# Eclectic-Sheep/sheeprl

Hardware: NVIDIA H100
Metric: Dreamer-V3 train-steps/sec (S, bs16 seq64 horizon15, 64x64x3 obs) (higher is better)
Workload: dtype f32

## Files before the change

include/b200rl.h:

```cpp
#ifndef B200RL_H_
#define B200RL_H_

#include <cuda_runtime_api.h>

#ifdef __cplusplus
extern "C" {
#endif

const char* b200rl_last_error(void);
int b200rl_abi_version(void);
const char* b200rl_build_arch(void);
int b200rl_device_check(void);

int b200rl_gemm_f32(const float* A, const float* B, float* C, const float* bias, int M, int N, int K, int lda, int ldb,
                    int ldc, int transA, int transB, int accumulate, cudaStream_t stream);
int b200rl_set_matmul_precision(int tf32_passes);
int b200rl_get_matmul_precision(void);
int b200rl_gemm_tc_supported(const float* A, const float* B, int M, int N, int K, int lda, int ldb, int transA,
                             int transB);
int b200rl_gemm_tc(const float* A, const float* B, float* C, const float* bias, int M, int N, int K, int lda, int ldb,
                   int ldc, int transA, int transB, int accumulate, cudaStream_t stream);
int b200rl_tf32_split(const float* X, float* Xhi, float* Xlo, long long n, cudaStream_t stream);
int b200rl_tf32_split_t(const float* W, float* Thi, float* Tlo, int rows, int cols, long long ldw, long long ldt,
                        cudaStream_t stream);
int b200rl_gemm_tc_presplit_supported(const float* A, const float* Bhi, const float* Blo, int M, int N, int K, int lda,
                                      int ldb);
int b200rl_gemm_tc_presplit(const float* A, const float* Bhi, const float* Blo, float* C, const float* bias, int M, int N,
                            int K, int lda, int ldb, int ldc, int accumulate, cudaStream_t stream);
int b200rl_gemm_ln_supported(const float* A, const float* W, int M, int N, int K, int lda, int ldw, int mode);
int b200rl_gemm_ln(const float* A, const float* W, int M, int N, int K, int lda, int ldw, const float* gamma,
                   const float* beta, float eps, int act, float* pre, long long ldpre, float* out, long long ldout,
                   int mode, const float* h_prev, long long ldh, float* h_out, long long ldho, float* h_out2,
                   long long ldho2, cudaStream_t stream);
int b200rl_gemm_ln_presplit_supported(const float* A, const float* Whi, const float* Wlo, int M, int N, int K, int lda,
                                      int ldw, int mode);
int b200rl_gemm_ln_presplit(const float* A, const float* Whi, const float* Wlo, int M, int N, int K, int lda, int ldw,
                            const float* gamma, const float* beta, float eps, int act, float* pre, long long ldpre,
                            float* out, long long ldout, int mode, const float* h_prev, long long ldh, float* h_out,
                            long long ldho, float* h_out2, long long ldho2, cudaStream_t stream);
int b200rl_ln_act_route(int C, long long ld0, long long ld1, long long ld2, const float* p0, const float* p1,
                        const float* p2, const float* gamma, const float* beta);
int b200rl_ln_act_fwd(const float* X, const float* gamma, const float* beta, float* Y, long long M, int C,
                      long long ldx, long long ldy, float eps, int act, cudaStream_t stream);
int b200rl_ln_act_bwd(const float* X, const float* gamma, const float* beta, const float* dY, float* dX, float* dgamma,
                      float* dbeta, long long M, int C, long long ldx, long long lddy, long long lddx, float eps,
                      int act, int accumulate, cudaStream_t stream);
int b200rl_col_sum(const float* X, float* out, long long M, int C, long long ldx, int accumulate, cudaStream_t stream);

int b200rl_obs_prep(const void* obs_nchw, int is_uint8, float* out_nhwc, long long NB, int C, int HW,
                    cudaStream_t stream);
int b200rl_transpose_batched(const float* X, float* Y, int NB, int a, int b, cudaStream_t stream);
int b200rl_transpose2d(const float* X, float* Y, int rows, int cols, long long ldx, long long ldy, cudaStream_t stream);
int b200rl_conv_down(const float* big, const float* W, float* small_, int NB, int h, int w, int Cs, int Cb,
                     cudaStream_t stream);
int b200rl_conv_up(const float* small_, const float* W, float* big, const float* bias, int NB, int h, int w, int Cs,
                   int Cb, cudaStream_t stream);
int b200rl_conv_wgrad(const float* small_, const float* big, float* dW, int NB, int h, int w, int Cs, int Cb,
// ... 224 lines not shown
```

sheeprl_b200/csrc/gemm_tc.cu:

```cuda
#include <cuda.h>
#include <cudaTypedefs.h>

#include <mutex>
#include <unordered_map>

#include "common.cuh"

namespace {

constexpr int BM = 128, BK = 32;
constexpr int NTHREADS = 384;
constexpr int NSPLIT_THREADS = 96;
constexpr int NCONS_WARPS = 8;
constexpr int PRODUCER_REGS = 56, CONSUMER_REGS = 224;
template <int PASSES, bool PRESPLIT> __host__ __device__ constexpr int b_buffers() { return PRESPLIT ? (PASSES == 3 ? 2 : 1) : 3; }
template <int BN, int PASSES, bool PRESPLIT> constexpr int stages_for() {
  return (227 * 1024 - 1024 - 256) / ((BM + b_buffers<PASSES, PRESPLIT>() * BN) * BK * (int)sizeof(float));
}

__device__ __forceinline__ uint32_t smem_u32(const void* p) { return (uint32_t)__cvta_generic_to_shared(p); }

__device__ __forceinline__ void mbar_init(uint64_t* bar, uint32_t count) {
  asm volatile("mbarrier.init.shared::cta.b64 [%0], %1;" ::"r"(smem_u32(bar)), "r"(count) : "memory");
}
__device__ __forceinline__ void mbar_expect_tx(uint64_t* bar, uint32_t bytes) {
  asm volatile("mbarrier.arrive.expect_tx.shared::cta.b64 _, [%0], %1;" ::"r"(smem_u32(bar)), "r"(bytes) : "memory");
}
__device__ __forceinline__ void mbar_arrive(uint64_t* bar) {
  asm volatile("mbarrier.arrive.shared::cta.b64 _, [%0];" ::"r"(smem_u32(bar)) : "memory");
}
__device__ __forceinline__ bool mbar_try_wait(uint64_t* bar, uint32_t parity) {
  uint32_t ok;
  asm volatile(
      "{\n\t"
      ".reg .pred p;\n\t"
      "mbarrier.try_wait.parity.shared::cta.b64 p, [%1], %2;\n\t"
      "selp.u32 %0, 1, 0, p;\n\t"
      "}"
// ... 479 lines not shown
  *bw = w < 128 ? w : 128;
  int rest = 128 / *bw;
  *bh = h < rest ? h : rest;
  *bn = rest / *bh;
  return (w % *bw == 0) && (h % *bh == 0) && (*bw * *bh * *bn == 128) && (NB % *bn == 0);
}

static unsigned persistent_grid_y(int tiles, unsigned gz) {
  const long long total = (long long)tiles * gz;
  if (total <= 2LL * kNumSMs) return (unsigned)tiles;
  unsigned gy = kNumSMs / gz;
  if (gy < 1) gy = 1;
  return gy < (unsigned)tiles ? gy : (unsigned)tiles;
}

__device__ __forceinline__ float tf32_hi(float x) { return __uint_as_float(__float_as_uint(x) & 0xffffe000u); }
__device__ __forceinline__ void store_split(float* P, float* L, long long i, float v) {
  if (L) { const float h = tf32_hi(v); P[i] = h; L[i] = v - h; }
  else P[i] = v;
}

__global__ void tf32_split_kernel(const float* __restrict__ X, float* __restrict__ H, float* __restrict__ L, long long n) {
  const long long i = ((long long)blockIdx.x * blockDim.x + threadIdx.x) * 4;
  if (i + 4 <= n && !((reinterpret_cast<uintptr_t>(X) | reinterpret_cast<uintptr_t>(H) | reinterpret_cast<uintptr_t>(L)) & 15)) {
    const float4 v = *reinterpret_cast<const float4*>(X + i);
    const float4 h = make_float4(tf32_hi(v.x), tf32_hi(v.y), tf32_hi(v.z), tf32_hi(v.w));
    *reinterpret_cast<float4*>(H + i) = h;
    *reinterpret_cast<float4*>(L + i) = make_float4(v.x - h.x, v.y - h.y, v.z - h.z, v.w - h.w);
  } else {
    for (long long j = i; j < i + 4 && j < n; ++j) store_split(H, L, j, X[j]);
  }
}

__global__ void tf32_split_t_kernel(const float* __restrict__ W, float* __restrict__ H, float* __restrict__ L, int rows,
                                    int cols, long long ldw, long long ldt) {
  __shared__ float t[32][33];
  const int c0 = blockIdx.x * 32, r0 = blockIdx.y * 32;
  for (int j = threadIdx.y; j < 32; j += blockDim.y) {
    const int r = r0 + j, c = c0 + threadIdx.x;
    t[j][threadIdx.x] = (r < rows && c < cols) ? W[(long long)r * ldw + c] : 0.f;
  }
  __syncthreads();
  for (int j = threadIdx.y; j < 32; j += blockDim.y) {
    const int c = c0 + j, r = r0 + threadIdx.x;
    if (c < cols && r < ldt) store_split(H, L, (long long)c * ldt + r, t[threadIdx.x][j]);
  }
}

__global__ void conv_pack_down_kernel(const float* __restrict__ W, float* __restrict__ P, float* __restrict__ L, int Cs,
                                      int Cb) {
  const long long idx = (long long)blockIdx.x * blockDim.x + threadIdx.x;
  if (idx >= (long long)Cs * Cb * 16) return;
  const int cb = (int)(idx % Cb);
  const int tap = (int)((idx / Cb) % 16);
  const int cs = (int)(idx / ((long long)Cb * 16));
  store_split(P, L, idx, W[((long long)cs * Cb + cb) * 16 + tap]);
}
__global__ void conv_pack_up_kernel(const float* __restrict__ W, float* __restrict__ P, float* __restrict__ L, int Cs,
                                    int Cb) {
  const long long idx = (long long)blockIdx.x * blockDim.x + threadIdx.x;
  if (idx >= (long long)Cs * Cb * 16) return;
  const int cs = (int)(idx % Cs);
  const int t = (int)((idx / Cs) % 4);
  const int cb = (int)((idx / ((long long)Cs * 4)) % Cb);
  const int par = (int)(idx / ((long long)Cs * 4 * Cb));
  const int py = par >> 1, px = par & 1;
// ... 170 lines not shown
  RL_CHECK_ARG(W && Whi && Wlo, "null pointer");
  return conv_pack_impl(W, Whi, Wlo, mode_up, Cs, Cb, st);
}
extern "C" int b200rl_conv_down_tc(const float* big, const float* Wpacked, float* small_, int NB, int h, int w, int Cs,
                                   int Cb, cudaStream_t st) {
  RL_CHECK_ARG(big && Wpacked && small_, "null pointer");
  RL_CHECK_ARG(b200rl_conv_tc_supported(0, NB, h, w, Cs, Cb), "shape not eligible for the tensor-core conv path");
  return launch_conv(MODE_DOWN, big, Wpacked, nullptr, small_, nullptr, NB, h, w, Cb, Cs, st);
}
extern "C" int b200rl_conv_up_tc(const float* small_, const float* Wpacked, float* big, const float* bias, int NB, int h,
                                 int w, int Cs, int Cb, cudaStream_t st) {
  RL_CHECK_ARG(big && Wpacked && small_, "null pointer");
  RL_CHECK_ARG(b200rl_conv_tc_supported(1, NB, h, w, Cs, Cb), "shape not eligible for the tensor-core conv path");
  return launch_conv(MODE_UP, small_, Wpacked, nullptr, big, bias, NB, h, w, Cs, Cb, st);
}
extern "C" int b200rl_conv_down_tc_presplit(const float* big, const float* Whi, const float* Wlo, float* small_, int NB,
                                            int h, int w, int Cs, int Cb, cudaStream_t st) {
  RL_CHECK_ARG(big && Whi && Wlo && small_, "null pointer");
  RL_CHECK_ARG(b200rl_conv_tc_supported(0, NB, h, w, Cs, Cb), "shape not eligible for the tensor-core conv path");
  return launch_conv(MODE_DOWN, big, Whi, Wlo, small_, nullptr, NB, h, w, Cb, Cs, st);
}
extern "C" int b200rl_conv_up_tc_presplit(const float* small_, const float* Whi, const float* Wlo, float* big,
                                          const float* bias, int NB, int h, int w, int Cs, int Cb, cudaStream_t st) {
  RL_CHECK_ARG(big && Whi && Wlo && small_, "null pointer");
  RL_CHECK_ARG(b200rl_conv_tc_supported(1, NB, h, w, Cs, Cb), "shape not eligible for the tensor-core conv path");
  return launch_conv(MODE_UP, small_, Whi, Wlo, big, bias, NB, h, w, Cs, Cb, st);
}

extern "C" int b200rl_tf32_split(const float* X, float* Xhi, float* Xlo, long long n, cudaStream_t st) {
  RL_CHECK_ARG(X && Xhi && Xlo, "null pointer");
  RL_CHECK_ARG(n >= 0, "negative length");
  if (n == 0) return B200RL_OK;
  tf32_split_kernel<<<ceil_div((n + 3) / 4, 256), 256, 0, st>>>(X, Xhi, Xlo, n);
  RL_CHECK_LAUNCH();
  return B200RL_OK;
}
extern "C" int b200rl_tf32_split_t(const float* W, float* Thi, float* Tlo, int rows, int cols, long long ldw, long long ldt,
                                   cudaStream_t st) {
  RL_CHECK_ARG(W && Thi && Tlo, "null pointer");
  RL_CHECK_ARG(rows > 0 && cols > 0 && ldw >= cols && ldt >= rows, "bad transposed-split geometry");
  dim3 grid(ceil_div(cols, 32), ceil_div(ldt, 32));
  tf32_split_t_kernel<<<grid, dim3(32, 8), 0, st>>>(W, Thi, Tlo, rows, cols, ldw, ldt);
  RL_CHECK_LAUNCH();
  return B200RL_OK;
}

extern "C" int b200rl_gemm_tc_supported(const float* A, const float* B, int M, int N, int K, int lda, int ldb,
                                        int transA, int transB) {
  (void)transA; (void)transB;
  if (M < 32 || N < 48 || K < 32) return 0;
  if ((lda & 3) || (ldb & 3)) return 0;
  if ((reinterpret_cast<uintptr_t>(A) & 15) || (reinterpret_cast<uintptr_t>(B) & 15)) return 0;
  return 1;
}

namespace {
struct FusedTail { float* part; int ks, mpad, ldw; };

int gemm_tc_impl(const float* A, const float* B, const float* Blo, float* C, const float* bias, int M, int N, int K,
                 int lda, int ldb, int ldc, int transA, int transB, int accumulate, cudaStream_t st, FusedTail* fused) {
  RL_CHECK_ARG(A && B && (C || fused), "null pointer");
  RL_CHECK_ARG(b200rl_gemm_tc_supported(A, B, M, N, K, lda, ldb, transA, transB), "shape not eligible for the tensor-core path");
  RL_CHECK_ARG(!Blo || (transB && !(reinterpret_cast<uintptr_t>(Blo) & 15)), "pre-split B must be 16-byte aligned [N][K] planes");
  const int BN = (N <= 64) ? 64 : 128;
  CUtensorMap ma, mb, mb2;
  if (!transA) { if (int rc = get_map(A, M, K, lda, BM, &ma)) return rc; }
// ... 249 lines not shown
```

sheeprl_b200/engine.py:

```python
from __future__ import annotations

import math
from typing import Dict, Mapping, Optional, Sequence

import torch

from sheeprl_b200.params import FlatGroup

ACT_NONE, ACT_SILU = 0, 1
TWOHOT_LOW, TWOHOT_HIGH = -20.0, 20.0


def decoder_channels(cfg, in_channels: int, cnn_dims: Optional[Mapping[str, int]] = None) -> int:
    a = cfg.algo
    dec = list(a.cnn_keys.decoder or [])
    if dec == list(a.cnn_keys.encoder or []):
        return in_channels
    missing = [k for k in dec if k not in (cnn_dims or {})]
    if missing:
        raise ValueError(f"the channel count of the decoded image key(s) {missing} is not known (pass cnn_dims)")
    return sum(int(cnn_dims[k]) for k in dec)


def check_decoder_keys(cfg) -> None:
# ... 89 lines not shown
    return wm, actor, critic, dict(chans=chans, dch=dch, E=E, Ev=Ev, stages=stages)


def _check_supported_modules(cfg) -> None:
    a, w = cfg.algo, cfg.algo.world_model
    blocks = {"algo": a, "encoder": w.encoder, "observation_model": w.observation_model, "reward_model": w.reward_model,
              "discount_model": w.discount_model, "transition_model": w.transition_model,
              "representation_model": w.representation_model, "recurrent_model": w.recurrent_model, "actor": a.actor,
              "critic": a.critic}
    for name, blk in blocks.items():
        for key in ("dense_act", "cnn_act"):
            v = blk.get(key, None)
            if v is not None and not str(v).endswith("SiLU"):
                raise NotImplementedError(f"{name}.{key} = {v}: only torch.nn.SiLU is built")
        for key in ("layer_norm", "mlp_layer_norm", "cnn_layer_norm"):
            v = blk.get(key, None)
            if v is not None and "LayerNorm" not in str(v.get("cls", "LayerNorm")):
                raise NotImplementedError(f"{name}.{key}.cls = {v.get('cls')}: only the LayerNorm variants are built")
    for name in ("reward_model", "discount_model"):
        blk = blocks[name]
        if int(blk.get("dense_units", a.dense_units)) != int(a.dense_units) or int(blk.get("mlp_layers", a.mlp_layers)) != int(a.mlp_layers):
            raise NotImplementedError(f"world_model.{name}: dense_units / mlp_layers must equal algo.dense_units / algo.mlp_layers")
    if int(w.observation_model.get("cnn_channels_multiplier", w.encoder.cnn_channels_multiplier)) != int(w.encoder.cnn_channels_multiplier):
        raise NotImplementedError("observation_model.cnn_channels_multiplier must equal encoder.cnn_channels_multiplier")
    for name in ("actor", "critic"):
        blk = blocks[name]
        if int(blk.get("dense_units", a.dense_units)) != int(a.dense_units) or int(blk.get("mlp_layers", a.mlp_layers)) != int(a.mlp_layers):
            raise NotImplementedError(f"algo.{name}: dense_units / mlp_layers must equal algo.dense_units / algo.mlp_layers")


FUSED_DENSE_MAX_ROWS = 4096


def dense_ln_act(ops, x, W, gamma, beta, eps, act, out, pre=None, scratch=None):
    if x.shape[0] <= FUSED_DENSE_MAX_ROWS and ops.gemm_ln_supported(x, W):
        ops.gemm_ln_act(x, W, gamma, beta, eps, act, out, pre)
        return
    tmp = pre if pre is not None else scratch
    ops.gemm(x, W, tmp, False, True)
    ops.ln_act_fwd(tmp, gamma, beta, eps, act, out)


class _MLP:

    def __init__(self, eng, group: FlatGroup, prefix: str, in_dim: int, hidden: int, n_hidden: int,
                 out_dim: Optional[int], rows: int, eps: float, tag: str, train: bool):
        self.eng, self.g, self.prefix = eng, group, prefix
        self.in_dim, self.hidden, self.n_hidden, self.out_dim, self.eps = in_dim, hidden, n_hidden, out_dim, eps
        self.rows = rows
        new = eng._buf
        self.pre = [new(f"{tag}.pre{i}", rows, hidden) for i in range(n_hidden)]
        self.act = [new(f"{tag}.act{i}", rows, hidden) for i in range(n_hidden)]
        self.out = new(f"{tag}.out", rows, out_dim) if out_dim is not None else None
        if train:
            self.dact = new(f"{tag}.dact", rows, hidden)
            self.dpre = new(f"{tag}.dpre", rows, hidden)

    def W(self, i):
        return self.g.views[f"{self.prefix}{3 * i}.weight"]

    def forward(self, x: torch.Tensor, group: Optional[FlatGroup] = None, M: Optional[int] = None):
        ops = self.eng.ops
        g = group or self.g
        M = x.shape[0] if M is None else M
        cur = x
        for i in range(self.n_hidden):
            dense_ln_act(ops, cur, g.views[f"{self.prefix}{3 * i}.weight"], g.views[f"{self.prefix}{3 * i + 1}.weight"],
                         g.views[f"{self.prefix}{3 * i + 1}.bias"], self.eps, ACT_SILU, self.act[i][:M], self.pre[i][:M])
            cur = self.act[i][:M]
        if self.out_dim is None:
            return cur
        j = 3 * self.n_hidden
# ... 79 lines not shown
        self.Z, self.R = self.S * self.D, w.recurrent_model.recurrent_state_size
        self.L = self.Z + self.R
        self.Rh = 0 if self.decoupled else self.R
        self.A = int(sum(self.actions_dim))
        self.du, self.nh = a.dense_units, a.mlp_layers
        self.Dx = w.recurrent_model.dense_units
        self.Dt, self.Dr = w.transition_model.hidden_size, w.representation_model.hidden_size
        self.eps = float(a.mlp_layer_norm.kw.eps)
        self.ceps = float(a.cnn_layer_norm.kw.eps)
        self.unimix = float(a.unimix)
        self.img = cfg.env.screen_size
        self.key = a.cnn_keys.encoder[0] if self.has_cnn else None
        self.bins_r, self.bins_c = w.reward_model.bins, a.critic.bins
        self.Cdec = decoder_channels(cfg, in_channels, self.cnn_dims) if self.has_cnn_dec else 0
        wm_s, ac_s, cr_s, meta = dv3_param_shapes(cfg, self.actions_dim, in_channels, self.is_continuous,
                                                  dict(zip(self.vec_keys, self.vec_dims)), self.cnn_dims)
        self.Ev = meta["Ev"]
        self.AW = 2 * self.A if self.is_continuous else self.A
        self.chans, self.dch, self.E, self.stages = meta["chans"], meta["dch"], meta["E"], meta["stages"]
        if groups is not None:
            self.wm, self.actor, self.critic, self.target = groups
        else:
            self.wm = FlatGroup(wm_s, device)
            self.actor = FlatGroup(ac_s, device)
            self.critic = FlatGroup(cr_s, device)
            self.target = FlatGroup(cr_s, device, with_optimizer=False)
        self.moments_state = torch.zeros(2, dtype=torch.float32, device=device)
        self.world_size = 1
        self.allreduce = None
        self.allgather = None
        self.allreduce_async = None
        self.allreduce_join = None
        self._bufs: Dict[str, torch.Tensor] = {}
        self._alloc()

    def _buf(self, name: str, *shape, dtype=torch.float32) -> torch.Tensor:
        assert name not in self._bufs, name
        t = torch.zeros(*shape, dtype=dtype, device=self.device)
        self._bufs[name] = t
        return t

    def _buf_ld4(self, name: str, rows: int, cols: int) -> torch.Tensor:
        return self._buf(name, rows, (cols + 3) // 4 * 4)[:, :cols]

    def _alloc(self):
        N, T, B, H, Z, R, L, A, E = self.N, self.T, self.B, self.H, self.Z, self.R, self.L, self.A, self.E
        b = self._buf
        img = self.img
        n_st = self.stages if self.has_cnn else 0
        self.x0 = b("x0", N, img, img, self.Cin) if self.has_cnn else None
        self.enc_y, self.enc_a = [], []
        s = img
        for i in range(n_st):
            s //= 2
            self.enc_y.append(b(f"enc_y{i}", N, s, s, self.chans[i + 1]))
            self.enc_a.append(b(f"enc_a{i}", N, s, s, self.chans[i + 1]))
        self.emb = b("emb", N, E) if self.has_cnn else None
        self.pe = b("pe", N, self.Dr)
        we, wo = self.cfg.algo.world_model.encoder, self.cfg.algo.world_model.observation_model
        if self.vec_keys:
            self.vx = b("vx", N, self.Dv)
            self.venc = _MLP(self, self.wm, "encoder.mlp_encoder.model._model.", self.Dv, we.dense_units, we.mlp_layers, None,
                             N, float(we.mlp_layer_norm.kw.eps), "venc", True)
            self.d_emb_vec = b("d_emb_vec", N, self.Ev)
        if self.has_vec_dec:
            self.vdec = _MLP(self, self.wm, "observation_model.mlp_decoder.model._model.", L, wo.dense_units, wo.mlp_layers,
# ... 368 lines not shown
                dv = self.vrecon[:, off:off + d]
                ops.gemm(dv, hid, self._gw(name + ".weight"), True, False)
                ops.col_sum(dv, self._gw(name + ".bias"))
                ops.gemm(dv, self._w(name + ".weight"), self.d_vdec_hidden, False, False, accumulate=True)
            self.vdec.backward(self.latent, self.d_vdec_hidden, self.d_latent, self.has_cnn_dec)

    def _cnn_decoder_backward(self):
        ops = self.ops
        st = self.stages
        wn = self._dec_names(st - 1)[0]
        d_big = self.recon
        ops.col_sum(d_big.view(-1, self.Cdec), self._gw(wn.replace(".weight", ".bias")))
        for i in reversed(range(st)):
            wn, gn, bn = self._dec_names(i)
            inp = self.dec_in if i == 0 else self.dec_a[i - 1]
            d_inp = self.d_dec_in if i == 0 else self.d_dec_a[i - 1]
            ops.conv_wgrad(inp, d_big, self._gw(wn))
            ops.conv_down(d_big, self._w(wn), d_inp)
            if i > 0:
                gn_p, bn_p = self._dec_names(i - 1)[1:]
                C = self.dch[i]
                d = d_inp.view(-1, C)
                ops.ln_act_bwd(self.dec_y[i - 1].view(-1, C), self._w(gn_p), self._w(bn_p), self.ceps, ACT_SILU, d, d,
                               self._gw(gn_p), self._gw(bn_p))
            d_big = d_inp
        C0 = self.dch[0]
        ops.transpose_batched(self.d_dec_in.view(self.N, 16, C0), self.d_dec_lin.view(self.N, C0, 16))
        p = "observation_model.cnn_decoder.model."
        ops.gemm(self.d_dec_lin, self.latent, self._gw(p + "0.weight"), True, False)
        ops.col_sum(self.d_dec_lin, self._gw(p + "0.bias"))
        ops.gemm(self.d_dec_lin, self._w(p + "0.weight"), self.d_latent, False, False)

    def _recurrent_forward(self, z, act, h_prev, x_pre, x_act, g_pre, g_ln, h_out, win_t=None, hx=None, h_next=None,
                           keep: bool = True):
        self._recurrent_input(z, act, x_pre, x_act, win_t, keep)
        return self._gru_forward(h_prev, x_act, g_pre, g_ln, h_out, hx, h_next, keep)

    def _recurrent_input(self, z, act, x_pre, x_act, win_t=None, keep: bool = True):
        ops, Z = self.ops, self.Z
        p = "rssm.recurrent_model."
        Win = self._w(p + "mlp._model.0.weight")
        fused_x = win_t is not None and ops.onehot_linear_ln_supported(win_t, x_act, x_pre if keep else None)
        if fused_x:
            ops.onehot_linear_ln(z, act, win_t, self._w(p + "mlp._model.1.weight"), self._w(p + "mlp._model.1.bias"),
                                 self.eps, x_act, self.S, self.D, pre=x_pre if keep else None)
        elif win_t is not None:
            ops.onehot_linear(z, act, win_t, x_pre, self.S, self.D)
        else:
            ops.gemm(z, Win[:, :Z], x_pre, False, True)
            ops.gemm(act, Win[:, Z:], x_pre, False, True, accumulate=True)
        if not fused_x:
            ops.ln_act_fwd(x_pre, self._w(p + "mlp._model.1.weight"), self._w(p + "mlp._model.1.bias"), self.eps,
                           ACT_SILU, x_act)

    def _gru_forward(self, h_prev, x_act, g_pre, g_ln, h_out, hx=None, h_next=None, keep: bool = True):
        ops, R = self.ops, self.R
        p = "rssm.recurrent_model."
        Wg = self._w(p + "rnn.linear.weight")
        if hx is not None and hx.shape[0] <= FUSED_DENSE_MAX_ROWS and ops.gemm_ln_supported(hx, Wg, 1):
            ops.gemm_ln_gru(hx, Wg, self._w(p + "rnn.layer_norm.weight"), self._w(p + "rnn.layer_norm.bias"), self.eps,
                            h_prev, h_out, h_next, g_pre if keep else None, g_ln if keep else None)
            return True
        if hx is not None:
            ops.gemm(hx, Wg, g_pre, False, True)
        else:
            ops.gemm(h_prev, Wg[:, :R], g_pre, False, True, accumulate=x_act is None)
            if x_act is not None:
                ops.gemm(x_act, Wg[:, R:], g_pre, False, True, accumulate=True)
        ops.ln_act_fwd(g_pre, self._w(p + "rnn.layer_norm.weight"), self._w(p + "rnn.layer_norm.bias"), self.eps,
                       ACT_NONE, g_ln)
        ops.gru_gate_fwd(g_ln, h_prev, h_out)
        return False

    def _recurrent_backward(self, g_ln, h_prev, g_pre, x_pre, dh, d_g_ln, d_g_pre, d_x_act, d_x_pre, dh_prev, dz,
                            da=None):
        ops, Z, R = self.ops, self.Z, self.R
        p = "rssm.recurrent_model."
        Win, Wg = self._w(p + "mlp._model.0.weight"), self._w(p + "rnn.linear.weight")
        self._gru_backward(g_ln, h_prev, g_pre, dh, d_g_ln, d_g_pre, dh_prev)
        ops.gemm(d_g_pre, Wg[:, R:], d_x_act, False, False)
        ops.ln_act_bwd(x_pre, self._w(p + "mlp._model.1.weight"), self._w(p + "mlp._model.1.bias"), self.eps, ACT_SILU,
                       d_x_act, d_x_pre, None, None)
        ops.gemm(d_x_pre, Win[:, :Z], dz, False, False)
        if da is not None:
            ops.gemm(d_x_pre, Win[:, Z:], da, False, False)

    def _gru_backward(self, g_ln, h_prev, g_pre, dh, d_g_ln, d_g_pre, dh_prev):
        ops = self.ops
        p = "rssm.recurrent_model.rnn."
        ops.gru_gate_bwd(g_ln, h_prev, dh, d_g_ln, dh_prev)
        ops.ln_act_bwd(g_pre, self._w(p + "layer_norm.weight"), self._w(p + "layer_norm.bias"), self.eps, ACT_NONE,
                       d_g_ln, d_g_pre, None, None)
        ops.gemm(d_g_pre, self._w(p + "linear.weight")[:, :self.R], dh_prev, False, False, accumulate=True)

    def _transition_forward(self, h, tr_pre, tr_act, raw, keep: bool = True):
        ops = self.ops
        p = "rssm.transition_model._model."
        dense_ln_act(ops, h, self._w(p + "0.weight"), self._w(p + "1.weight"), self._w(p + "1.bias"), self.eps, ACT_SILU,
                     tr_act, tr_pre if keep else None, scratch=tr_pre)
        ops.gemm(tr_act, self._w(p + "3.weight"), raw, False, True, bias=self._w(p + "3.bias"))

    def _transition_backward(self, raw, tr_pre, dz, dmix, d_raw, d_tr_act, d_tr_pre, dh, ln_grads: bool = False):
        ops = self.ops
        p = "rssm.transition_model._model."
        ops.cat_sample_bwd(raw, dz, dmix, self.unimix, self.S, self.D, d_raw)
        ops.gemm(d_raw, self._w(p + "3.weight"), d_tr_act, False, False)
        ops.ln_act_bwd(tr_pre, self._w(p + "1.weight"), self._w(p + "1.bias"), self.eps, ACT_SILU, d_tr_act, d_tr_pre,
                       self._gw(p + "1.weight") if ln_grads else None, self._gw(p + "1.bias") if ln_grads else None)
        ops.gemm(d_tr_pre, self._w(p + "0.weight"), dh, False, False, accumulate=True)

    def _posterior_forward(self, h, rp_pre, rp_act, raw, noise, z_out, mix_out=None):
        ops, R = self.ops, self.R
        pr = "rssm.representation_model._model."
        if h is not None:
            ops.gemm(h, self._w(pr + "0.weight")[:, :R], rp_pre, False, True, accumulate=True)
        ops.ln_act_fwd(rp_pre, self._w(pr + "1.weight"), self._w(pr + "1.bias"), self.eps, ACT_SILU, rp_act)
        ops.gemm(rp_act, self._w(pr + "3.weight"), raw, False, True, bias=self._w(pr + "3.bias"))
        ops.cat_sample(raw, noise, self.unimix, self.S, self.D, z_out, mix_out)

    def _scan_forward(self, first: torch.Tensor):
        ops, B, Z, R = self.ops, self.B, self.Z, self.R
        ops.tanh_fwd(self._w("rssm.initial_recurrent_state").view(1, R), self.h0)
        self._transition_forward(self.h0, self.init_tr_pre, self.init_tr_act, self.init_raw)
        ops.cat_sample(self.init_raw, None, self.unimix, self.S, self.D, self.z0)
        if self.decoupled:
            self._scan_forward_decoupled(first)
        elif self.fused_scan:
            self._scan_forward_fused(first)
        for t in (() if self.fused_scan or self.decoupled else range(self.T)):
            s = slice(t * B, (t + 1) * B)
            f = first[s]
            if t == 0:
                zp, hp = self.zero_z, self.zero_h
# ... 196 lines not shown

    def _wm_buckets(self):
        off = self.wm.offsets
        b_enc = off["rssm.initial_recurrent_state"]
        tail = [v for k, v in off.items() if not (k.startswith("encoder.") or k.startswith("rssm."))]
        return b_enc, min(tail)

    def _optimizer_step(self, name: str, g: FlatGroup, max_norm: float, ocfg, slot: int, reduced: bool = False):
        ops = self.ops
        if self.allreduce is not None and not reduced:
            self.allreduce(g.grad, name)
        ops.sumsq(g.grad, self.normsq[name])
        g.step += 1
        ops.increment(g.step_t)
        b1, b2 = ocfg.betas
        opt = getattr(g, "optimizer", None)
        lr = opt.lr if opt is not None else float(ocfg.lr)
        ops.adam_step(g.flat, g.grad, g.exp_avg, g.exp_avg_sq, self.normsq[name], max_norm, lr,
                      float(b1), float(b2), float(ocfg.eps), g.step_t, self.norms[slot: slot + 1],
                      **g.adam_kwargs(ocfg.get("weight_decay", 0.0)))

    def _actor_heads(self, hidden: torch.Tensor, raw_out: torch.Tensor, actor: Optional[FlatGroup] = None):
        actor = actor or self.actor
        if self.is_continuous:
            self.ops.gemm(hidden, actor.views["mlp_heads.0.weight"], raw_out, False, True,
                          bias=actor.views["mlp_heads.0.bias"])
            return
        off = 0
        for i, ad in enumerate(self.actions_dim):
            self.ops.gemm(hidden, actor.views[f"mlp_heads.{i}.weight"], raw_out[:, off:off + ad], False, True,
                          bias=actor.views[f"mlp_heads.{i}.bias"])
            off += ad

    def _imagine(self, actor: Optional[FlatGroup] = None, actor_mlp: Optional["_MLP"] = None):
        ops, N, Z, R, H = self.ops, self.N, self.Z, self.R, self.H
        actor = actor or self.actor
        am = actor_mlp or self.actor_mlp
        Win = self._w("rssm.recurrent_model.mlp._model.0.weight")
        gather = ops.onehot_linear_supported(self.S, self.D, self.A, Win.shape[0])
        if gather:
            if getattr(self, "_win_t", None) is None:
                self._win_t = torch.empty(Win.shape[1], Win.shape[0], dtype=torch.float32, device=self.device)
            ops.transpose2d(Win, self._win_t)
        h_staged = False
        for i in range(H + 1):
            rows = slice(i * N, (i + 1) * N)
            if i > 0:
                prev, cur = self.traj[i - 1], self.traj[i]
                if self.is_continuous:
                    j = i - 1
                    x_pre, hx, g_pre, g_ln = self.c_x_pre[j], self.c_hx[j], self.c_g_pre[j], self.c_g_ln[j]
                    tr_pre, tr_act, raw = self.c_tr_pre[j], self.c_tr_act[j], self.c_raw[j]
                else:
                    x_pre, hx, g_pre, g_ln = self.i_x_pre, self.i_hx, self.i_g_pre, self.i_g_ln
                    tr_pre, tr_act, raw = self.i_tr_pre, self.i_tr_act, self.i_raw
                if not h_staged:
                    ops.copy(prev[:, Z:], hx[:, :R])
                keep = self.is_continuous
                h_next = None
                if i < H:
                    h_next = (self.c_hx[i] if self.is_continuous else hx)[:, :R]
                h_staged = self._recurrent_forward(prev[:, :Z], self.actions[i - 1], prev[:, Z:], x_pre, hx[:, R:], g_pre,
                                                   g_ln, cur[:, Z:], win_t=self._win_t if gather else None, hx=hx,
                                                   h_next=h_next, keep=keep) and h_next is not None
                self._transition_forward(cur[:, Z:], tr_pre, tr_act, raw, keep=keep)
                ops.cat_sample(raw, self.noise_img_state[i - 1], self.unimix, self.S, self.D, cur[:, :Z])
            x = self.traj[i]
            cur_in = x
            for l in range(am.n_hidden):
                dense_ln_act(ops, cur_in, am.W(l), actor.views[f"model._model.{3 * l + 1}.weight"],
                             actor.views[f"model._model.{3 * l + 1}.bias"], self.eps, ACT_SILU, am.act[l][rows],
                             am.pre[l][rows])
                cur_in = am.act[l][rows]
            if not self.is_continuous:
                off, done = 0, True
                for k, ad in enumerate(self.actions_dim):
                    Wh = actor.views[f"mlp_heads.{k}.weight"]
                    done = done and ops.head_sample_supported(cur_in, Wh)
                if done:
                    for k, ad in enumerate(self.actions_dim):
                        ops.head_sample(cur_in, actor.views[f"mlp_heads.{k}.weight"], actor.views[f"mlp_heads.{k}.bias"],
                                        self.noise_img_action[i, :, off:off + ad], self.unimix,
                                        self.actor_raw[rows, off:off + ad], self.actions[i, :, off:off + ad])
                        off += ad
                    continue
            self._actor_heads(cur_in, self.actor_raw[rows], actor)
            if self.is_continuous:
                ac = self.cfg.algo.actor
                ops.cont_action_fwd(self.actor_raw[rows], self.noise_img_action[i], self.actions[i], self.act_ent[rows],
                                    float(ac.min_std), float(ac.max_std), float(ac.init_std), float(ac.action_clip))
                continue
            off = 0
            for k, ad in enumerate(self.actions_dim):
                ops.cat_sample(self.actor_raw[rows, off:off + ad], self.noise_img_action[i, :, off:off + ad],
                               self.unimix, 1, ad, self.actions[i, :, off:off + ad])
                off += ad


    def _continuous_policy_gradient(self, c_logit, critics):
        ops, N, H, Z, R, L = self.ops, self.N, self.H, self.Z, self.R, self.L
        a = self.cfg.algo
        ac = a.actor
        M1, M0 = (H + 1) * N, H * N
        traj2, d_traj2 = self.traj.view(M1, L), self.d_traj.view(M1, L)
        for j, (mlp, v_logits, values, lam, moments, share, r_logits, rows) in enumerate(critics):
# ... 109 lines not shown
```

sheeprl_b200/lib.py:

```python
from __future__ import annotations

import ctypes
import os
import re
from typing import Optional, Sequence

import torch

_HERE = os.path.dirname(os.path.abspath(__file__))
LIB_PATH = os.path.join(_HERE, "libb200rl.so")
HEADER_PATH = os.path.join(os.path.dirname(_HERE), "include", "b200rl.h")

_lib = None

PRESPLIT_MIN_ROWS = 4096


class B200RLError(RuntimeError):
    pass


_SCALARS = {"int": ctypes.c_int, "long long": ctypes.c_longlong, "unsigned int": ctypes.c_uint,
            "unsigned long long": ctypes.c_ulonglong, "float": ctypes.c_float}

# ... 68 lines not shown


def _p(t: Optional[torch.Tensor]):
    return None if t is None else t.data_ptr()


def _ld(t: Optional[torch.Tensor]) -> int:
    if t is None:
        return 0
    if t.dim() == 1:
        assert t.numel() <= 1 or t.stride(0) == 1, "1-D views must be contiguous"
        return max(t.numel(), 1)
    assert t.dim() == 2, f"expected a 2-D view, got {tuple(t.shape)}"
    assert t.shape[1] == 1 or t.stride(1) == 1, f"inner stride must be 1, got {t.stride()}"
    return t.stride(0) if t.shape[0] > 1 else max(t.stride(0), t.shape[1])


def _f32(*ts):
    for t in ts:
        if t is not None:
            assert t.dtype == torch.float32 and t.is_cuda, (t.dtype, t.device)


def _struct(name: str, typedef: str, exclude=()):
    fields = _STRUCTS[typedef]
    pointers = tuple(n for n, t in fields if t is ctypes.c_void_p and n not in exclude)
    return type(name, (ctypes.Structure,), {"_fields_": fields, "POINTERS": pointers})


RssmScanArgs = _struct("RssmScanArgs", "b200rl_rssm_scan_args", exclude=("workspace",))
RssmScanGrads = _struct("RssmScanGrads", "b200rl_rssm_scan_grads")
GruScanArgs = _struct("GruScanArgs", "b200rl_gru_scan_args", exclude=("workspace",))
GruScanGrads = _struct("GruScanGrads", "b200rl_gru_scan_grads")


class CudaOps:
    name = "cuda"

    def __init__(self, device="cuda"):
        if not torch.cuda.is_available():
            raise B200RLError("no CUDA device visible: the B200 engine has no CPU fallback")
        self.lib = load_library()
        self.device = torch.device(device)
        if self.device.index is not None:
            torch.cuda.set_device(self.device)
        if self.lib.b200rl_device_check() != 0:
            raise B200RLError(self.lib.b200rl_last_error().decode())
        self.launches = 0
        self.use_tc = os.environ.get("B200RL_DISABLE_TC", "0") != "1"
        self._pack_bufs = {}
        self._scratch_bufs = {}

    def _st(self):
        return torch.cuda.current_stream().cuda_stream

    def _ck(self, rc: int, launches: int = 1):
        self.launches += launches
        if rc != 0:
            raise B200RLError(self.lib.b200rl_last_error().decode())

    def set_matmul_precision(self, precision: str) -> None:
        p = str(precision).lower()
        if p not in ("highest", "high", "medium"):
            raise ValueError(f"float32_matmul_precision must be highest / high / medium, got {precision}")
        self._ck(self.lib.b200rl_set_matmul_precision(3 if p == "highest" else 1), 0)

    def matmul_precision(self) -> str:
        return "highest" if self.lib.b200rl_get_matmul_precision() == 3 else "high"

    def gemm(self, A, B, C, transA: bool, transB: bool, bias=None, accumulate: bool = False):
        _f32(A, B, C, bias)
        M, N = C.shape
        K = A.shape[0] if transA else A.shape[1]
        assert (A.shape[1] if transA else A.shape[0]) == M, (A.shape, C.shape, transA)
        assert (B.shape[0] if transB else B.shape[1]) == N and (B.shape[1] if transB else B.shape[0]) == K, \
            (A.shape, B.shape, C.shape, transA, transB)
        if (not transA and M >= PRESPLIT_MIN_ROWS and self.use_tc
                and self.lib.b200rl_gemm_tc_supported(_p(A), _p(B), M, N, K, _ld(A), _ld(B), 0, int(transB))):
            hi, lo, ld = self._planes(B, transB, N, K)
            self._ck(self.lib.b200rl_gemm_tc_presplit(_p(A), _p(hi), _p(lo), _p(C), _p(bias), M, N, K, _ld(A), ld, _ld(C),
                                                      int(accumulate), self._st()))
            return
        self._ck(self.lib.b200rl_gemm_f32(_p(A), _p(B), _p(C), _p(bias), M, N, K, _ld(A), _ld(B), _ld(C), int(transA),
                                          int(transB), int(accumulate), self._st()))

    def _planes(self, B, transB: bool, N: int, K: int):
        ldb = _ld(B)
        ld = ldb if transB else (K + 3) // 4 * 4
        buf = self._scratch("b_planes", 2 * N * ld)
        hi, lo = buf[:N * ld], buf[N * ld:2 * N * ld]
        if transB:
            self._ck(self.lib.b200rl_tf32_split(_p(B), _p(hi), _p(lo), (N - 1) * ldb + K, self._st()))
        else:
            self._ck(self.lib.b200rl_tf32_split_t(_p(B), _p(hi), _p(lo), K, N, ldb, ld, self._st()))
        return hi, lo, ld

    def gemm_ln_supported(self, A, W, mode: int = 0) -> bool:
        M, K = A.shape
        return self.use_tc and bool(self.lib.b200rl_gemm_ln_supported(_p(A), _p(W), M, W.shape[0], K, _ld(A), _ld(W),
                                                                     mode))

    def gemm_ln_act(self, A, W, gamma, beta, eps: float, act: int, out, pre=None):
        _f32(A, W, gamma, beta, out, pre)
        M, K = A.shape
        N = W.shape[0]
        assert W.shape[1] == K and out.shape == (M, N)
        self._ck(self.lib.b200rl_gemm_ln(_p(A), _p(W), M, N, K, _ld(A), _ld(W), _p(gamma), _p(beta), eps, act, _p(pre),
                                         _ld(pre), _p(out), _ld(out), 0, None, 0, None, 0, None, 0, self._st()), 2)

    def gemm_ln_gru(self, A, W, gamma, beta, eps: float, h_prev, h_out, h_out2=None, g_pre=None, g_ln=None):
        _f32(A, W, gamma, beta, h_prev, h_out, h_out2, g_pre, g_ln)
        M, K = A.shape
        N = W.shape[0]
        assert W.shape[1] == K and h_prev.shape == (M, N // 3) and h_out.shape == (M, N // 3)
        self._ck(self.lib.b200rl_gemm_ln(_p(A), _p(W), M, N, K, _ld(A), _ld(W), _p(gamma), _p(beta), eps, 0, _p(g_pre),
                                         _ld(g_pre), _p(g_ln), _ld(g_ln), 1, _p(h_prev), _ld(h_prev), _p(h_out),
                                         _ld(h_out), _p(h_out2), _ld(h_out2), self._st()), 2)

    def _scratch(self, slot: str, numel: int) -> torch.Tensor:
        buf = self._scratch_bufs.get(slot)
        if buf is None or buf.numel() < numel:
            buf = torch.empty(numel, dtype=torch.float32, device=self.device)
            self._scratch_bufs[slot] = buf
        return buf

    def col_sum(self, X, out, accumulate: bool = False):
        _f32(X, out)
        self._ck(self.lib.b200rl_col_sum(_p(X), _p(out), X.shape[0], X.shape[1], _ld(X), int(accumulate), self._st()))

    def ln_act_fwd(self, X, gamma, beta, eps: float, act: int, Y):
        _f32(X, gamma, beta, Y)
        self._ck(self.lib.b200rl_ln_act_fwd(_p(X), _p(gamma), _p(beta), _p(Y), X.shape[0], X.shape[1], _ld(X), _ld(Y),
                                            eps, act, self._st()))

    def ln_act_bwd(self, X, gamma, beta, eps: float, act: int, dY, dX, dgamma, dbeta, accumulate: bool = False):
        _f32(X, gamma, beta, dY, dX, dgamma, dbeta)
        self._ck(self.lib.b200rl_ln_act_bwd(_p(X), _p(gamma), _p(beta), _p(dY), _p(dX), _p(dgamma), _p(dbeta),
                                            X.shape[0], X.shape[1], _ld(X), _ld(dY), _ld(dX), eps, act,
                                            int(accumulate), self._st()))

    def obs_prep(self, obs, out):
        assert obs.is_cuda and obs.is_contiguous() and out.is_contiguous()
        assert obs.dtype in (torch.uint8, torch.float32), obs.dtype
        NB, C, H, W = obs.shape
        self._ck(self.lib.b200rl_obs_prep(_p(obs), int(obs.dtype == torch.uint8), _p(out), NB, C, H * W, self._st()))

    def transpose_batched(self, X, Y):
        _f32(X, Y)
        assert X.is_contiguous() and Y.is_contiguous()
        NB, a, b = X.shape
# ... 569 lines not shown
```

Measured before the change: 60.34.

## Pre-split rollout weights into TF32 planes once per imagination with batched split kernel

Before each imagination rollout, the GRU, transition and actor weights are split into TF32 hi/lo planes using a single multi-range split kernel launch. The per-step GEMM and fused GEMM+LN calls in the 15-step rollout then use the presplit entry points, so they no longer split the weights on every call. The cost is extra plane buffers and one split launch per rollout. The planes must be recomputed whenever the weights change, which holds here because the split runs at the start of every _imagine call.

After: 61.19, median of 6. 1.4% higher.

```diff
diff --git a/include/b200rl.h b/include/b200rl.h
--- a/include/b200rl.h
+++ b/include/b200rl.h
@@ -23,6 +23,12 @@
 int b200rl_tf32_split(const float* X, float* Xhi, float* Xlo, long long n, cudaStream_t stream);
 int b200rl_tf32_split_t(const float* W, float* Thi, float* Tlo, int rows, int cols, long long ldw, long long ldt,
                         cudaStream_t stream);
+typedef struct b200rl_tf32_range {
+  const float* X;
+  float *hi, *lo;
+  long long n;
+} b200rl_tf32_range;
+int b200rl_tf32_split_ranges(const b200rl_tf32_range* ranges, int count, cudaStream_t stream);
 int b200rl_gemm_tc_presplit_supported(const float* A, const float* Bhi, const float* Blo, int M, int N, int K, int lda,
                                       int ldb);
 int b200rl_gemm_tc_presplit(const float* A, const float* Bhi, const float* Blo, float* C, const float* bias, int M, int N,
diff --git a/sheeprl_b200/csrc/gemm_tc.cu b/sheeprl_b200/csrc/gemm_tc.cu
--- a/sheeprl_b200/csrc/gemm_tc.cu
+++ b/sheeprl_b200/csrc/gemm_tc.cu
@@ -4,6 +4,7 @@
 #include <mutex>
 #include <unordered_map>
 
+#include "b200rl.h"
 #include "common.cuh"
 
 namespace {
@@ -549,6 +550,32 @@
   }
 }
 
+constexpr int kMaxSplitRanges = 8;
+struct SplitRanges {
+  const float* X[kMaxSplitRanges];
+  float* H[kMaxSplitRanges];
+  float* L[kMaxSplitRanges];
+  long long n[kMaxSplitRanges];
+  int first[kMaxSplitRanges + 1];
+  int count;
+};
+
+__global__ void tf32_split_ranges_kernel(const SplitRanges r) {
+  int k = 0;
+  while (k + 1 < r.count && (int)blockIdx.x >= r.first[k + 1]) ++k;
+  const long long i = ((long long)(blockIdx.x - r.first[k]) * blockDim.x + threadIdx.x) * 4, n = r.n[k];
+  const float* X = r.X[k];
+  float *H = r.H[k], *L = r.L[k];
+  if (i + 4 <= n && !((reinterpret_cast<uintptr_t>(X) | reinterpret_cast<uintptr_t>(H) | reinterpret_cast<uintptr_t>(L)) & 15)) {
+    const float4 v = *reinterpret_cast<const float4*>(X + i);
+    const float4 h = make_float4(tf32_hi(v.x), tf32_hi(v.y), tf32_hi(v.z), tf32_hi(v.w));
+    *reinterpret_cast<float4*>(H + i) = h;
+    *reinterpret_cast<float4*>(L + i) = make_float4(v.x - h.x, v.y - h.y, v.z - h.z, v.w - h.w);
+  } else {
+    for (long long j = i; j < i + 4 && j < n; ++j) store_split(H, L, j, X[j]);
+  }
+}
+
 __global__ void tf32_split_t_kernel(const float* __restrict__ W, float* __restrict__ H, float* __restrict__ L, int rows,
                                     int cols, long long ldw, long long ldt) {
   __shared__ float t[32][33];
@@ -785,6 +812,26 @@
   RL_CHECK_ARG(n >= 0, "negative length");
   if (n == 0) return B200RL_OK;
   tf32_split_kernel<<<ceil_div((n + 3) / 4, 256), 256, 0, st>>>(X, Xhi, Xlo, n);
+  RL_CHECK_LAUNCH();
+  return B200RL_OK;
+}
+extern "C" int b200rl_tf32_split_ranges(const b200rl_tf32_range* ranges, int count, cudaStream_t st) {
+  RL_CHECK_ARG(ranges && count >= 1 && count <= kMaxSplitRanges, "1 to 8 ranges");
+  SplitRanges r = {};
+  r.count = count;
+  long long blocks = 0;
+  for (int k = 0; k < count; ++k) {
+    const b200rl_tf32_range& g = ranges[k];
+    RL_CHECK_ARG(g.n >= 0, "negative length");
+    RL_CHECK_ARG(g.n == 0 || (g.X && g.hi && g.lo), "null pointer");
+    r.X[k] = g.X; r.H[k] = g.hi; r.L[k] = g.lo; r.n[k] = g.n;
+    r.first[k] = (int)blocks;
+    blocks += ceil_div((g.n + 3) / 4, 256);
+    RL_CHECK_ARG(blocks < (1LL << 31), "ranges too long for one launch");
+  }
+  r.first[count] = (int)blocks;
+  if (blocks == 0) return B200RL_OK;
+  tf32_split_ranges_kernel<<<(unsigned)blocks, 256, 0, st>>>(r);
   RL_CHECK_LAUNCH();
   return B200RL_OK;
 }
diff --git a/sheeprl_b200/engine.py b/sheeprl_b200/engine.py
--- a/sheeprl_b200/engine.py
+++ b/sheeprl_b200/engine.py
@@ -145,12 +145,16 @@
 FUSED_DENSE_MAX_ROWS = 4096
 
 
-def dense_ln_act(ops, x, W, gamma, beta, eps, act, out, pre=None, scratch=None):
+def with_planes(planes) -> dict:
+    return {} if planes is None else {"planes": planes}
+
+
+def dense_ln_act(ops, x, W, gamma, beta, eps, act, out, pre=None, scratch=None, planes=None):
     if x.shape[0] <= FUSED_DENSE_MAX_ROWS and ops.gemm_ln_supported(x, W):
-        ops.gemm_ln_act(x, W, gamma, beta, eps, act, out, pre)
+        ops.gemm_ln_act(x, W, gamma, beta, eps, act, out, pre, **with_planes(planes))
         return
     tmp = pre if pre is not None else scratch
-    ops.gemm(x, W, tmp, False, True)
+    ops.gemm(x, W, tmp, False, True, **with_planes(planes))
     ops.ln_act_fwd(tmp, gamma, beta, eps, act, out)
 
 
@@ -296,6 +300,7 @@
         self.allreduce_async = None
         self.allreduce_join = None
         self._bufs: Dict[str, torch.Tensor] = {}
+        self._plane_bufs = {}
         self._alloc()
 
     def _buf(self, name: str, *shape, dtype=torch.float32) -> torch.Tensor:
@@ -730,9 +735,9 @@
         ops.gemm(self.d_dec_lin, self._w(p + "0.weight"), self.d_latent, False, False)
 
     def _recurrent_forward(self, z, act, h_prev, x_pre, x_act, g_pre, g_ln, h_out, win_t=None, hx=None, h_next=None,
-                           keep: bool = True):
+                           keep: bool = True, planes=None):
         self._recurrent_input(z, act, x_pre, x_act, win_t, keep)
-        return self._gru_forward(h_prev, x_act, g_pre, g_ln, h_out, hx, h_next, keep)
+        return self._gru_forward(h_prev, x_act, g_pre, g_ln, h_out, hx, h_next, keep, planes)
 
     def _recurrent_input(self, z, act, x_pre, x_act, win_t=None, keep: bool = True):
         ops, Z = self.ops, self.Z
@@ -751,16 +756,18 @@
             ops.ln_act_fwd(x_pre, self._w(p + "mlp._model.1.weight"), self._w(p + "mlp._model.1.bias"), self.eps,
                            ACT_SILU, x_act)
 
-    def _gru_forward(self, h_prev, x_act, g_pre, g_ln, h_out, hx=None, h_next=None, keep: bool = True):
+    def _gru_forward(self, h_prev, x_act, g_pre, g_ln, h_out, hx=None, h_next=None, keep: bool = True, planes=None):
         ops, R = self.ops, self.R
         p = "rssm.recurrent_model."
         Wg = self._w(p + "rnn.linear.weight")
+        Wg_planes = (planes or {}).get(p + "rnn.linear.weight")
         if hx is not None and hx.shape[0] <= FUSED_DENSE_MAX_ROWS and ops.gemm_ln_supported(hx, Wg, 1):
             ops.gemm_ln_gru(hx, Wg, self._w(p + "rnn.layer_norm.weight"), self._w(p + "rnn.layer_norm.bias"), self.eps,
-                            h_prev, h_out, h_next, g_pre if keep else None, g_ln if keep else None)
+                            h_prev, h_out, h_next, g_pre if keep else None, g_ln if keep else None,
+                            **with_planes(Wg_planes))
             return True
         if hx is not None:
-            ops.gemm(hx, Wg, g_pre, False, True)
+            ops.gemm(hx, Wg, g_pre, False, True, **with_planes(Wg_planes))
         else:
             ops.gemm(h_prev, Wg[:, :R], g_pre, False, True, accumulate=x_act is None)
             if x_act is not None:
@@ -791,12 +798,14 @@
                        d_g_ln, d_g_pre, None, None)
         ops.gemm(d_g_pre, self._w(p + "linear.weight")[:, :self.R], dh_prev, False, False, accumulate=True)
 
-    def _transition_forward(self, h, tr_pre, tr_act, raw, keep: bool = True):
+    def _transition_forward(self, h, tr_pre, tr_act, raw, keep: bool = True, planes=None):
         ops = self.ops
         p = "rssm.transition_model._model."
+        pl = planes or {}
         dense_ln_act(ops, h, self._w(p + "0.weight"), self._w(p + "1.weight"), self._w(p + "1.bias"), self.eps, ACT_SILU,
-                     tr_act, tr_pre if keep else None, scratch=tr_pre)
-        ops.gemm(tr_act, self._w(p + "3.weight"), raw, False, True, bias=self._w(p + "3.bias"))
+                     tr_act, tr_pre if keep else None, scratch=tr_pre, planes=pl.get(p + "0.weight"))
+        ops.gemm(tr_act, self._w(p + "3.weight"), raw, False, True, bias=self._w(p + "3.bias"),
+                 **with_planes(pl.get(p + "3.weight")))
 
     def _transition_backward(self, raw, tr_pre, dz, dmix, d_raw, d_tr_act, d_tr_pre, dh, ln_grads: bool = False):
         ops = self.ops
@@ -1059,10 +1068,27 @@
                           bias=actor.views[f"mlp_heads.{i}.bias"])
             off += ad
 
+    def _rollout_planes(self, actor: FlatGroup) -> Dict[str, tuple]:
+        split = getattr(self.ops, "tf32_split_ranges", None)
+        if split is None:
+            return {}
+        names = ("rssm.recurrent_model.rnn.linear.weight", "rssm.transition_model._model.0.weight",
+                 "rssm.transition_model._model.3.weight")
+        srcs = [(n, self._w(n)) for n in names] + [(actor, actor.flat)]
+        for key, src in srcs:
+            if key not in self._plane_bufs:
+                self._plane_bufs[key] = (torch.empty_like(src), torch.empty_like(src))
+        split([(src, *self._plane_bufs[key]) for key, src in srcs])
+        planes = {n: self._plane_bufs[n] for n in names}
+        hi, lo = self._plane_bufs[actor]
+        planes.update(zip(actor.shapes, zip(actor._views(hi).values(), actor._views(lo).values())))
+        return planes
+
     def _imagine(self, actor: Optional[FlatGroup] = None, actor_mlp: Optional["_MLP"] = None):
         ops, N, Z, R, H = self.ops, self.N, self.Z, self.R, self.H
         actor = actor or self.actor
         am = actor_mlp or self.actor_mlp
+        planes = self._rollout_planes(actor)
         Win = self._w("rssm.recurrent_model.mlp._model.0.weight")
         gather = ops.onehot_linear_supported(self.S, self.D, self.A, Win.shape[0])
         if gather:
@@ -1089,15 +1115,15 @@
                     h_next = (self.c_hx[i] if self.is_continuous else hx)[:, :R]
                 h_staged = self._recurrent_forward(prev[:, :Z], self.actions[i - 1], prev[:, Z:], x_pre, hx[:, R:], g_pre,
                                                    g_ln, cur[:, Z:], win_t=self._win_t if gather else None, hx=hx,
-                                                   h_next=h_next, keep=keep) and h_next is not None
-                self._transition_forward(cur[:, Z:], tr_pre, tr_act, raw, keep=keep)
+                                                   h_next=h_next, keep=keep, planes=planes) and h_next is not None
+                self._transition_forward(cur[:, Z:], tr_pre, tr_act, raw, keep=keep, planes=planes)
                 ops.cat_sample(raw, self.noise_img_state[i - 1], self.unimix, self.S, self.D, cur[:, :Z])
             x = self.traj[i]
             cur_in = x
             for l in range(am.n_hidden):
                 dense_ln_act(ops, cur_in, am.W(l), actor.views[f"model._model.{3 * l + 1}.weight"],
                              actor.views[f"model._model.{3 * l + 1}.bias"], self.eps, ACT_SILU, am.act[l][rows],
-                             am.pre[l][rows])
+                             am.pre[l][rows], planes=planes.get(f"model._model.{3 * l}.weight"))
                 cur_in = am.act[l][rows]
             if not self.is_continuous:
                 off, done = 0, True
diff --git a/sheeprl_b200/lib.py b/sheeprl_b200/lib.py
--- a/sheeprl_b200/lib.py
+++ b/sheeprl_b200/lib.py
@@ -124,6 +124,7 @@
 RssmScanGrads = _struct("RssmScanGrads", "b200rl_rssm_scan_grads")
 GruScanArgs = _struct("GruScanArgs", "b200rl_gru_scan_args", exclude=("workspace",))
 GruScanGrads = _struct("GruScanGrads", "b200rl_gru_scan_grads")
+Tf32Range = _struct("Tf32Range", "b200rl_tf32_range")
 
 
 class CudaOps:
@@ -160,13 +161,19 @@
     def matmul_precision(self) -> str:
         return "highest" if self.lib.b200rl_get_matmul_precision() == 3 else "high"
 
-    def gemm(self, A, B, C, transA: bool, transB: bool, bias=None, accumulate: bool = False):
+    def gemm(self, A, B, C, transA: bool, transB: bool, bias=None, accumulate: bool = False, planes=None):
         _f32(A, B, C, bias)
         M, N = C.shape
         K = A.shape[0] if transA else A.shape[1]
         assert (A.shape[1] if transA else A.shape[0]) == M, (A.shape, C.shape, transA)
         assert (B.shape[0] if transB else B.shape[1]) == N and (B.shape[1] if transB else B.shape[0]) == K, \
             (A.shape, B.shape, C.shape, transA, transB)
+        if planes is not None and not transA and transB and self.use_tc:
+            hi, lo = planes
+            if self.lib.b200rl_gemm_tc_presplit_supported(_p(A), _p(hi), _p(lo), M, N, K, _ld(A), _ld(hi)):
+                self._ck(self.lib.b200rl_gemm_tc_presplit(_p(A), _p(hi), _p(lo), _p(C), _p(bias), M, N, K, _ld(A),
+                                                          _ld(hi), _ld(C), int(accumulate), self._st()))
+                return
         if (not transA and M >= PRESPLIT_MIN_ROWS and self.use_tc
                 and self.lib.b200rl_gemm_tc_supported(_p(A), _p(B), M, N, K, _ld(A), _ld(B), 0, int(transB))):
             hi, lo, ld = self._planes(B, transB, N, K)
@@ -187,27 +194,46 @@
             self._ck(self.lib.b200rl_tf32_split_t(_p(B), _p(hi), _p(lo), K, N, ldb, ld, self._st()))
         return hi, lo, ld
 
+    def tf32_split_ranges(self, ranges):
+        arr = (Tf32Range * len(ranges))()
+        for r, (X, hi, lo) in zip(arr, ranges):
+            _f32(X, hi, lo)
+            assert X.is_contiguous() and hi.is_contiguous() and lo.is_contiguous() and hi.numel() == lo.numel() == X.numel()
+            r.X, r.hi, r.lo, r.n = _p(X), _p(hi), _p(lo), X.numel()
+        self._ck(self.lib.b200rl_tf32_split_ranges(ctypes.addressof(arr), len(ranges), self._st()))
+
     def gemm_ln_supported(self, A, W, mode: int = 0) -> bool:
         M, K = A.shape
         return self.use_tc and bool(self.lib.b200rl_gemm_ln_supported(_p(A), _p(W), M, W.shape[0], K, _ld(A), _ld(W),
                                                                      mode))
 
-    def gemm_ln_act(self, A, W, gamma, beta, eps: float, act: int, out, pre=None):
+    def _gemm_ln(self, A, W, planes, mode: int, *tail):
+        M, K = A.shape
+        N = W.shape[0]
+        if planes is not None:
+            hi, lo = planes
+            if self.lib.b200rl_gemm_ln_presplit_supported(_p(A), _p(hi), _p(lo), M, N, K, _ld(A), _ld(hi), mode):
+                self._ck(self.lib.b200rl_gemm_ln_presplit(_p(A), _p(hi), _p(lo), M, N, K, _ld(A), _ld(hi), *tail,
+                                                          self._st()), 2)
+                return
+        self._ck(self.lib.b200rl_gemm_ln(_p(A), _p(W), M, N, K, _ld(A), _ld(W), *tail, self._st()), 2)
+
+    def gemm_ln_act(self, A, W, gamma, beta, eps: float, act: int, out, pre=None, planes=None):
         _f32(A, W, gamma, beta, out, pre)
         M, K = A.shape
         N = W.shape[0]
         assert W.shape[1] == K and out.shape == (M, N)
-        self._ck(self.lib.b200rl_gemm_ln(_p(A), _p(W), M, N, K, _ld(A), _ld(W), _p(gamma), _p(beta), eps, act, _p(pre),
-                                         _ld(pre), _p(out), _ld(out), 0, None, 0, None, 0, None, 0, self._st()), 2)
-
-    def gemm_ln_gru(self, A, W, gamma, beta, eps: float, h_prev, h_out, h_out2=None, g_pre=None, g_ln=None):
+        self._gemm_ln(A, W, planes, 0, _p(gamma), _p(beta), eps, act, _p(pre), _ld(pre), _p(out), _ld(out), 0, None, 0,
+                      None, 0, None, 0)
+
+    def gemm_ln_gru(self, A, W, gamma, beta, eps: float, h_prev, h_out, h_out2=None, g_pre=None, g_ln=None,
+                    planes=None):
         _f32(A, W, gamma, beta, h_prev, h_out, h_out2, g_pre, g_ln)
         M, K = A.shape
         N = W.shape[0]
         assert W.shape[1] == K and h_prev.shape == (M, N // 3) and h_out.shape == (M, N // 3)
-        self._ck(self.lib.b200rl_gemm_ln(_p(A), _p(W), M, N, K, _ld(A), _ld(W), _p(gamma), _p(beta), eps, 0, _p(g_pre),
-                                         _ld(g_pre), _p(g_ln), _ld(g_ln), 1, _p(h_prev), _ld(h_prev), _p(h_out),
-                                         _ld(h_out), _p(h_out2), _ld(h_out2), self._st()), 2)
+        self._gemm_ln(A, W, planes, 1, _p(gamma), _p(beta), eps, 0, _p(g_pre), _ld(g_pre), _p(g_ln), _ld(g_ln), 1,
+                      _p(h_prev), _ld(h_prev), _p(h_out), _ld(h_out), _p(h_out2), _ld(h_out2))
 
     def _scratch(self, slot: str, numel: int) -> torch.Tensor:
         buf = self._scratch_bufs.get(slot)
```
